# DrStiev/raytracing_rust

Hardware: AMD Instinct MI355X
Metric: Msamples/s (W×H×spp/s) + wall-clock to PPM, final_scene 1920×1080×1000spp (higher is better)
Workload: dtype f32; 1 GPU; final_scene 1920x1080x1000spp; per_gpu=1920x1080x1000spp-equivalent (tiles t % 1 == rank), scene_seed=1, render_seed=42, max_depth=50, flags=1

## Files before the change

### raytracing_rust_amd/csrc/rtmi_bvh_coop.hpp

```cpp
#pragma once
#include "rtmi_bvh.hpp"
#include "rtmi_rng.hpp"

#define COOP_NONE 0xffffffffu
#define RTMI_COOP_DUMMY_WORDS 128u
#define COOP_SENTINEL 0xffffffffffffffffull
__device__ __forceinline__ uint32_t f2sort(float f) {
    const uint32_t u = __float_as_uint(f);
    return (u & 0x80000000u) ? ~u : (u | 0x80000000u);
}
__device__ __forceinline__ float sort2f(uint32_t s) {
    return __uint_as_float((s & 0x80000000u) ? (s & 0x7fffffffu) : ~s);
}

struct CoopLds {
    uint32_t cap;
    bool ext, insd;
    constexpr uint32_t ctx() const { return 2u * cap; }
    constexpr uint32_t best() const { return ctx() + 64u * 12u; }
    constexpr uint32_t dummy() const { return best() + 128u; }
    constexpr uint32_t ring() const { return dummy() + RTMI_COOP_DUMMY_WORDS; }
    constexpr uint32_t park() const { return ring() + (ext ? 0u : RTMI_RNG_RING_WORDS); }
    constexpr uint32_t words() const { return park() + (insd ? RTMI_COOP_PARK_WORDS : 0u); }
};

struct CoopWork {
    uint32_t *wlds;
    int cap;
    uint2 *spill;
    int spill_cap;
};

#define RTMI_COOP_INLINE __forceinline__
template <bool PROF, bool EXT, bool W4, bool INST, bool QU = false>
__device__ __forceinline__ void coop_bvh_query(const DevScene &sc, int root, bool gated, float scale, bool active, const RayF &R,
                                               float time, float q_min, float q_max, const CoopWork &cw,
                                               bool &have, float &t_out, int &pf_out, bool &overflow,
                                               unsigned long long *prof, int slot) {
    const int lane = threadIdx.x & 63;
    uint32_t *wlds = cw.wlds;
    const int cap = cw.cap;
    uint2 *pool = reinterpret_cast<uint2 *>(wlds);
    const CoopLds lds{(uint32_t)cap, false, false};
    float4 *ctx = reinterpret_cast<float4 *>(wlds + lds.ctx());
    unsigned long long *best = reinterpret_cast<unsigned long long *>(wlds + lds.best());

    const unsigned long long m_act = __ballot(active);
    have = false;
    if (m_act == 0ull) return;
    best[lane] = COOP_SENTINEL;
    uint32_t cur = COOP_NONE;
    int ray = 0, cray = -1, aray = -1;
    float tent = 0.0f;
    RayF W;
    W.o = f3(0, 0, 0); W.d = f3(0, 0, 1); W.inv_d = f3(0, 0, 0); W.a = 1.0f; W.inv_a = 1.0f;
    float wtime = 0.0f, wqmin = 0.0f, wqmax = 0.0f, wmabs = 0.0f;
    if (active) {
        ctx[lane * 3 + 0] = make_float4(R.o.x, R.o.y, R.o.z, time);
        ctx[lane * 3 + 1] = make_float4(R.d.x, R.d.y, R.d.z, QU ? R.inv_a : q_min);
        ctx[lane * 3 + 2] = make_float4(R.inv_d.x, R.inv_d.y, R.inv_d.z, q_max);
        cur = (uint32_t)root; ray = lane; cray = lane;
        tent = q_min;
        W.o = R.o; W.d = R.d; W.inv_d = R.inv_d;
        wtime = time; wqmin = q_min; wqmax = q_max;
        if (QU) { W.a = R.a; W.inv_a = R.inv_a; aray = lane; }
        wmabs = scale * (1.0f / 8192.0f) *
                fminf(fminf(__builtin_fabsf(W.inv_d.x), __builtin_fabsf(W.inv_d.y)), __builtin_fabsf(W.inv_d.z));
    }
    if (QU) wqmin = q_min;
    int top = 0, gtop = 0;
    __builtin_amdgcn_fence(__ATOMIC_RELEASE, "wavefront");
    __builtin_amdgcn_wave_barrier();

    uint32_t wch[4] = {0u, 0u, 0u, 0u};
    float wtn[4] = {0.0f, 0.0f, 0.0f, 0.0f};
    const auto visit4 = [&](float limit, uint32_t &wkeep, int &npush) {
        const uint32_t base = cur * 8u;
        const uint32_t sx = W.inv_d.x < 0.0f ? 3u : 0u, sy = W.inv_d.y < 0.0f ? 3u : 0u, sz = W.inv_d.z < 0.0f ? 3u : 0u;
        const float4 nx4 = sc.nodes4[base + sx], fx4 = sc.nodes4[base + 3u - sx];
        const float4 ny4 = sc.nodes4[base + 1u + sy], fy4 = sc.nodes4[base + 4u - sy];
        const float4 nz4 = sc.nodes4[base + 2u + sz], fz4 = sc.nodes4[base + 5u - sz];
        const float4 chf = sc.nodes4[base + 6u];
        const float anx[4] = {nx4.x, nx4.y, nx4.z, nx4.w}, afx[4] = {fx4.x, fx4.y, fx4.z, fx4.w};
        const float any_[4] = {ny4.x, ny4.y, ny4.z, ny4.w}, afy[4] = {fy4.x, fy4.y, fy4.z, fy4.w};
        const float anz[4] = {nz4.x, nz4.y, nz4.z, nz4.w}, afz[4] = {fz4.x, fz4.y, fz4.z, fz4.w};
        wch[0] = __float_as_uint(chf.x); wch[1] = __float_as_uint(chf.y); wch[2] = __float_as_uint(chf.z); wch[3] = __float_as_uint(chf.w);
        int nearest = -1;
        float tnear = RTMI_FLT_MAX;
        const float far0 = fminf(wqmax, limit);
#pragma unroll
        for (int c = 0; c < 4; c++) {
            const float tn = fmaxf(fmaxf(fmaxf(wqmin, (anx[c] - W.o.x) * W.inv_d.x), (any_[c] - W.o.y) * W.inv_d.y), (anz[c] - W.o.z) * W.inv_d.z);
            const float tf = fminf(fminf(fminf(far0, (afx[c] - W.o.x) * W.inv_d.x), (afy[c] - W.o.y) * W.inv_d.y), (afz[c] - W.o.z) * W.inv_d.z);
            wtn[c] = tn;
            const bool okc = !(tn > tf) && wch[c] != COOP_NONE;
            if (okc) wkeep |= 1u << c;
            if (okc && !(tn >= tnear)) { nearest = c; tnear = tn; }
        }
        if (nearest >= 0) { cur = wch[nearest]; tent = tnear; wkeep &= ~(1u << nearest); } else cur = COOP_NONE;
        npush = __popc(wkeep);
    };
    const auto publish4 = [&](uint32_t wkeep, int npush) {
        const unsigned long long b0 = __ballot((npush & 1) != 0), b1 = __ballot((npush & 2) != 0);
        const int before = (int)__builtin_amdgcn_mbcnt_hi((uint32_t)(b0 >> 32), __builtin_amdgcn_mbcnt_lo((uint32_t)b0, 0u)) +
                           2 * (int)__builtin_amdgcn_mbcnt_hi((uint32_t)(b1 >> 32), __builtin_amdgcn_mbcnt_lo((uint32_t)b1, 0u));
        int at = top + before;
        const int dummy = cap + (int)((lds.dummy() - lds.ctx()) / 2u) + lane;
#pragma unroll
        for (int c = 0; c < 4; c++) {
            const bool on = (wkeep & (1u << c)) != 0u;
            pool[on ? at : dummy] = make_uint2(((uint32_t)ray << 26) | wch[c], __float_as_uint(wtn[c]));
            at += on ? 1 : 0;
        }
        top += __popcll(b0) + 2 * __popcll(b1);
    };
    for (;;) {
    for (;;) {
        const bool needw = cur == COOP_NONE;
        const unsigned long long m_need = __ballot(needw);
        const int n_need = __popcll(m_need);
        if (top == 0 && n_need == 64) break;
        if (top > cap - (W4 ? 192 : 64)) {
            if (!EXT) overflow = true;
            break;
        }
        const int take = n_need < top ? n_need : top;
        {
            const int r = (int)__builtin_amdgcn_mbcnt_hi((uint32_t)(m_need >> 32), __builtin_amdgcn_mbcnt_lo((uint32_t)m_need, 0u));
            if (needw && r < take) {
                const int idx = top - 1 - r;
                const uint2 e = pool[idx];
                tent = __uint_as_float(e.y);
                cur = e.x & 0x03ffffffu;
                ray = (int)(e.x >> 26);
            }
        }
        top -= take;
        prof_tick<PROF>(prof, slot, cur != COOP_NONE);
        bool push = false;
        uint32_t push_ref = 0u;
        float push_t = 0.0f;
        int npush = 0;
        uint32_t wkeep = 0u;
        {
            if (cur != COOP_NONE && ray != cray) {
                const float4 c0 = ctx[ray * 3 + 0], c1 = ctx[ray * 3 + 1], c2 = ctx[ray * 3 + 2];
                W.o = f3(c0.x, c0.y, c0.z); wtime = c0.w;
                W.d = f3(c1.x, c1.y, c1.z);
                if (QU) W.inv_a = c1.w; else wqmin = c1.w;
                W.inv_d = f3(c2.x, c2.y, c2.z); wqmax = c2.w;
                wmabs = scale * (1.0f / 8192.0f) *
                        fminf(fminf(__builtin_fabsf(W.inv_d.x), __builtin_fabsf(W.inv_d.y)), __builtin_fabsf(W.inv_d.z));
                cray = ray;
            }
            const unsigned long long key = best[ray];
            const float bt = sort2f((uint32_t)(key >> 32));
            const float lim = bt + (__builtin_fabsf(bt) * (1.0f / 128.0f) + wmabs);
            const float limit = key != COOP_SENTINEL ? lim : RTMI_FLT_MAX;
            if (tent > limit) cur = COOP_NONE;
            if (W4 && !(cur & (1u << 25))) {
                visit4(limit, wkeep, npush);
            } else if (!W4 && !(cur & (1u << 25))) {
                const float4 *n = sc.nodes + (size_t)cur * 4;
                const float4 n0 = n[0], n1 = n[1], n2 = n[2], n3 = n[3];
                const uint32_t left = __float_as_uint(n3.z), right = __float_as_uint(n3.w);
                float tl, tr;
                bool vl = aabb_hit_t(n0.x, n0.y, n0.z, n0.w, n1.x, n1.y, W, wqmin, wqmax, tl);
                bool vr = aabb_hit_t(n1.z, n1.w, n2.x, n2.y, n2.z, n2.w, W, wqmin, wqmax, tr);
                vl = vl && !(tl > limit);
                vr = vr && !(tr > limit) && right != left;
                if (vl && vr) {
                    const bool lfirst = !(tr < tl);
                    push = true;
                    push_ref = lfirst ? right : left;
                    push_t = lfirst ? tr : tl;
                    cur = lfirst ? left : right;
                    tent = lfirst ? tl : tr;
                } else if (vl) { cur = left; tent = tl; }
                else if (vr) { cur = right; tent = tr; }
                else cur = COOP_NONE;
            }
        }
        if (cur != COOP_NONE && (cur & (1u << 25))) {
            {
                const int type = (int)((cur >> 22) & 7u);
                const int idx = (int)(cur & 0x003fffffu);
                float t;
                int pf;
                if (type <= RTMI_PRIM_MSPHERE && aray != ray) {
                    W.a = dot(W.d, W.d);
                    if (!QU) W.inv_a = 1.0f / W.a;
                    aray = ray;
                }
                bool hit;
                if (EXT && gated) {
                    const float4 *rec = sc.leaf_rec + (size_t)idx * 5;
                    const float4 A = rec[0], B = rec[1], M = rec[2], g0 = rec[3], g1 = rec[4];
                    hit = prim_test_vals<INST>(sc, type, idx, A, B, M.z, __float_as_uint(M.y), W, wtime, wqmin, wqmax, t, pf);
                    if (hit) hit = aabb_hit(g0.x, g0.y, g0.z, g1.x, g1.y, g1.z, W, wqmin, wqmax);
                } else {
                    hit = prim_test<INST>(sc, type, idx, W, wtime, wqmin, wqmax, t, pf);
                }
                if (hit) {
                    const unsigned long long k = ((unsigned long long)f2sort(t) << 32) | (unsigned long long)(0x7fffffffu - (uint32_t)pf);
                    atomicMin(&best[ray], k);
                }
                cur = COOP_NONE;
            }
        }
        if (W4) {
            if (__ballot(npush != 0) != 0ull) publish4(wkeep, npush);
        } else {
        const unsigned long long m_push = __ballot(push);
        if (push) {
            const int pos = top + (int)__builtin_amdgcn_mbcnt_hi((uint32_t)(m_push >> 32), __builtin_amdgcn_mbcnt_lo((uint32_t)m_push, 0u));
            pool[pos] = make_uint2(((uint32_t)ray << 26) | push_ref, __float_as_uint(push_t));
        }
        top += __popcll(m_push);
        }
        if (PROF && lane == 0) atomicMax(&prof[2 * 18], (unsigned long long)top);
        __builtin_amdgcn_fence(__ATOMIC_ACQ_REL, "wavefront");
        __builtin_amdgcn_wave_barrier();
    }
        if (!EXT) break;
        if (top > cap - (W4 ? 192 : 64)) {
            const int m = top - 64;
            if (gtop + m > cw.spill_cap) { overflow = true; break; }
            for (int i = lane; i < m; i += 64) cw.spill[gtop + i] = pool[i];
            const int rest = top - m;
            for (int base = 0; base < rest; base += 64) {
                const int i = base + lane;
                uint2 e = make_uint2(0u, 0u);
                if (i < rest) e = pool[m + i];
                __builtin_amdgcn_wave_barrier();
                if (i < rest) pool[i] = e;
            }
            gtop += m;
            top = rest;
        } else if (gtop > 0) {
            const int n = gtop < cap / 2 ? gtop : cap / 2;
            for (int i = lane; i < n; i += 64) pool[i] = cw.spill[gtop - n + i];
            gtop -= n;
            top = n;
        } else {
            break;
        }
        __builtin_amdgcn_fence(__ATOMIC_ACQ_REL, "wavefront");
        __builtin_amdgcn_wave_barrier();
    }
    __builtin_amdgcn_fence(__ATOMIC_ACQ_REL, "wavefront");
    __builtin_amdgcn_wave_barrier();
    if (active) {
        const unsigned long long key = best[lane];
        if (key != COOP_SENTINEL) {
            have = true;
            t_out = sort2f((uint32_t)(key >> 32));
            pf_out = (int)(0x7fffffffu - (uint32_t)key);
        }
    }
    __builtin_amdgcn_wave_barrier();
}

template <bool PROF, bool EXT, bool W4, bool INST, bool ONE = false, bool QU = false>
__device__ __forceinline__ bool geom_query_coop(const DevScene &sc, const rtmi_item &I, bool use_alt, bool active, const RayF &r,
                                                float time, float q_min, float q_max, const CoopWork &cw,
                                                float &t_out, int &pf_out, bool &overflow, unsigned long long *prof,
                                                int slot) {
    if (I.kind == RTMI_ITEM_BVH) {
        const bool enter = active && aabb_hit(I.root_min[0], I.root_min[1], I.root_min[2], I.root_max[0], I.root_max[1],
                                              I.root_max[2], r, q_min, q_max);
        bool have = false;
        static_assert(!ONE || (EXT && W4), "the one-tree form walks the gated 4-wide tree");
        if constexpr (ONE) {
            coop_bvh_query<PROF, EXT, W4, INST, QU>(sc, I.alt_first, true, I.scale, enter, r, time, q_min, q_max, cw, have, t_out, pf_out, overflow, prof, slot);
        } else {
        const bool alt = EXT && W4 && use_alt && I.alt_first >= 0;
        if (alt) coop_bvh_query<PROF, EXT, W4, INST, QU>(sc, I.alt_first, true, I.scale, enter, r, time, q_min, q_max, cw, have, t_out, pf_out, overflow, prof, slot);
        else coop_bvh_query<PROF, EXT, false, INST, QU>(sc, I.first, false, I.scale, enter, r, time, q_min, q_max, cw, have, t_out, pf_out, overflow, prof, slot);
        }
        return have;
    }
    float cl = q_max;
    bool any = false;
    if (active) {
        for (int k = 0; k < I.count; k++) {
            const int idx = I.first + k;
            float t;
            int pf;
            prof_tick<PROF>(prof, 13, true);
            if (prim_test_uniform<INST>(sc, idx, r, time, q_min, cl, t, pf)) { cl = t; any = true; pf_out = pf; }
        }
    }
    t_out = cl;
    return any;
}
```

### raytracing_rust_amd/csrc/rtmi_device.hip

```cpp
#include <hip/hip_runtime.h>

#include <dlfcn.h>
#include <time.h>

#include <algorithm>
#include <cmath>
#include <cstdio>
#include <cstdlib>
#include <cstring>
#include <limits>
#include <map>
#include <mutex>
#include <new>
#include <string>
#include <thread>
#include <utility>
#include <vector>

#include "rtmi.h"
#include "rtmi_math.h"

#include "rtmi_kernels.hpp"
#include "rtmi_render_launch.hpp"
#include "rtmi_probe_path_launch.hpp"
// ... 178 lines not shown
    if (d->max_bvh_depth > RTMI_MAX_BVH_DEPTH)
        return fail(RTMI_ERR_UNSUPPORTED, "BVH deeper than RTMI_MAX_BVH_DEPTH");
    if (d->n_prims >= (1u << 28)) return fail(RTMI_ERR_UNSUPPORTED, "too many primitives");
    if ((d->n_prims && (!d->prim_a || !d->prim_b || !d->prim_meta)) || (d->n_nodes && !d->nodes) || (d->n_xforms && !d->xforms) ||
        (d->n_materials && !d->materials) || (d->n_textures && !d->textures) || (d->n_perlin && !d->perlin) ||
        (d->n_images && !d->images) || (d->image_bytes && !d->image_data))
        return fail(RTMI_ERR_INVALID, "a non-zero count comes with a NULL array");
    auto prim_ok = [&](int64_t i) { return i >= 0 && (uint64_t)i < d->n_prims; };
    for (uint32_t i = 0; i < d->n_prims; i++) {
        const rtmi_prim_meta &m = d->prim_meta[i];
        if (m.type < 0 || m.type > RTMI_PRIM_CUBE) return fail(RTMI_ERR_INVALID, "bad primitive type");
        if (m.material < 0 || (uint32_t)m.material >= d->n_materials)
            return fail(RTMI_ERR_INVALID, "primitive material out of range");
        const uint32_t xfc = (m.flags >> RTMI_PRIMFLAG_XF_COUNT_SHIFT) & RTMI_PRIM_XF_MAX, xff = m.flags >> RTMI_PRIMFLAG_XF_FIRST_SHIFT;
        if (xfc != 0u && ((uint64_t)xff + xfc > d->n_xforms)) return fail(RTMI_ERR_INVALID, "primitive transform range out of bounds");
        for (uint32_t k = 0; k < xfc; k++)
            if (d->xforms[xff + k].kind > RTMI_XF_ROTATE_Z) return fail(RTMI_ERR_INVALID, "a gate or inner-medium record inside a primitive's transform chain");
    }
    for (uint32_t i = 0; i < d->n_xforms; i++)
        if (d->xforms[i].kind < RTMI_XF_TRANSLATE || d->xforms[i].kind > RTMI_XF_INNER_MEDIUM) return fail(RTMI_ERR_INVALID, "bad transform kind");
    for (uint32_t i = 0; i < d->n_nodes; i++) {
        const int32_t ch[2] = {d->nodes[i].left, d->nodes[i].right};
        for (int c = 0; c < 2; c++) {
            if (ch[c] >= 0) {
                if ((uint32_t)ch[c] >= d->n_nodes) return fail(RTMI_ERR_INVALID, "BVH child out of range");
            } else {
                uint32_t type = ((uint32_t)ch[c] >> 28) & 7u, idx = (uint32_t)ch[c] & 0x0fffffffu;
                if (type > RTMI_PRIM_CUBE || !prim_ok(idx)) return fail(RTMI_ERR_INVALID, "BVH leaf out of range");
                if ((int)type != d->prim_meta[idx].type) return fail(RTMI_ERR_INVALID, "BVH leaf type mismatch");
            }
        }
    }
    if (d->n_alt_nodes && !d->alt_nodes) return fail(RTMI_ERR_INVALID, "n_alt_nodes without alt_nodes");
    for (uint32_t i = 0; i < d->n_alt_nodes; i++)
        for (int c = 0; c < 4; c++) {
            const int32_t ch = d->alt_nodes[i].child[c];
            if (ch == RTMI_NO_CHILD) continue;
            if (ch >= 0) {
                if ((uint32_t)ch >= d->n_alt_nodes) return fail(RTMI_ERR_INVALID, "alternative tree child out of range");
            } else {
                const uint32_t type = ((uint32_t)ch >> 28) & 7u, idx = (uint32_t)ch & 0x0fffffffu;
                if (type > RTMI_PRIM_CUBE || !prim_ok(idx)) return fail(RTMI_ERR_INVALID, "alternative tree leaf out of range");
                if ((int)type != d->prim_meta[idx].type) return fail(RTMI_ERR_INVALID, "alternative tree leaf type mismatch");
            }
        }
    std::vector<uint8_t> seen_bin(d->n_nodes, 0), seen_alt(d->n_alt_nodes, 0);
    std::vector<std::pair<uint32_t, uint32_t>> todo;
    const auto walk = [&](bool alt, uint32_t root, uint32_t declared, const char *what) -> int {
        std::vector<uint8_t> &seen = alt ? seen_alt : seen_bin;
        todo.clear();
        todo.emplace_back(root, 1u);
        while (!todo.empty()) {
            const uint32_t n = todo.back().first, depth = todo.back().second;
            todo.pop_back();
            if (seen[n]) return fail(RTMI_ERR_INVALID, std::string(what) + ": a node is reached twice (cycle or shared subtree)");
            seen[n] = 1;
            if (depth > declared) return fail(RTMI_ERR_INVALID, std::string(what) + " is deeper than the declared depth");
            if (alt) {
                for (int c = 0; c < 4; c++) {
                    const int32_t ch = d->alt_nodes[n].child[c];
                    if (ch >= 0 && ch != RTMI_NO_CHILD) todo.emplace_back((uint32_t)ch, depth + 1u);
                }
            } else {
                const int32_t l = d->nodes[n].left, r = d->nodes[n].right;
                if (l >= 0) todo.emplace_back((uint32_t)l, depth + 1u);
                if (r >= 0 && r != l) todo.emplace_back((uint32_t)r, depth + 1u);
// ... 514 lines not shown
    hipStream_t stream = reinterpret_cast<hipStream_t>(stream_);
    if (s->busy_recorded) HIP_TRY(hipStreamWaitEvent(stream, s->busy.e, 0));
    BusyMark busy_mark{s, stream};

    DevParams P = dev_params(s, p);
    if (P.ntiles_local == 0) {
        if (stats) memset(stats, 0, sizeof(*stats));
        return RTMI_OK;
    }
    P.path_sig = reinterpret_cast<unsigned long long *>(p->path_sig);
    if (p->flags & RTMI_FLAG_PATH_SIG) {
        if (!p->path_sig) return fail(RTMI_ERR_INVALID, "RTMI_FLAG_PATH_SIG needs params.path_sig");
        HIP_TRY(hipMemsetAsync(P.path_sig, 0, (size_t)P.ntiles_local * 64 * sizeof(unsigned long long), stream));
    }

    uint32_t chunk_spp = 0, pass_ns = 0;
    rc = plan_and_reserve(s, p, P.ntiles_local, chunk_spp, pass_ns);
    if (rc) return rc;
    P.chunk_spp = chunk_spp;
    P.pass_stride = pass_ns;
    P.samples = s->samples.ptr;
    const DevCamera C = dev_camera(cam);

    if (stats) HIP_TRY(hipEventRecord(s->ev[0].e, stream));
    const bool fast = (p->flags & RTMI_FLAG_FAST_CULL) != 0u && boxes_valid(s, cam), sigf = (p->flags & RTMI_FLAG_PATH_SIG) != 0u;
    const size_t dyn_lds = (size_t)WAVES_PER_BLOCK * 2u * P.stack_depth * 64u * sizeof(uint32_t);
    const bool prof = (p->flags & RTMI_FLAG_PROFILE) != 0u, sync = (p->flags & RTMI_FLAG_SYNC) != 0u;
    if (prof) {
        if (!p->prof) return fail(RTMI_ERR_INVALID, "RTMI_FLAG_PROFILE needs params.prof");
        P.prof = reinterpret_cast<unsigned long long *>(p->prof);
        HIP_TRY(hipMemsetAsync(P.prof, 0, 2 * RTMI_PROF_SLOTS * sizeof(unsigned long long), stream));
    }
    const bool async = (p->flags & RTMI_FLAG_ASYNC) != 0u && !s->has_deferred;
    const bool coop_ok = s->meta.n_prims < (1u << 22) && s->meta.n_nodes < (1u << 25) && s->meta.n_alt_nodes < (1u << 25);
    const bool coop = fast && !sync && !async && coop_ok;
    if ((rc = begin_passes(s, stream))) return rc;
    bool ext = false;
    if ((rc = plan_traversal(s, p, coop, P, ext))) return rc;
    if (p->flags & (1u << 11)) {
        ext = true;
        P.coop_cap = 256u;
    }
    const uint32_t wps_req = (p->flags >> 8) & 7u;
    const bool inst = s->dev.has_prim_xf != 0u || s->dev.has_medium_outer != 0u;
    const uint32_t wps_run = (coop && !prof && !sigf && !inst && (wps_req == 3u || wps_req == 5u)) ? wps_req : (coop && prof ? 3u : 4u);
    const uint64_t run_slots = (uint64_t)(s->slots / 20) * 4u * wps_run;
    const bool bcoop = coop && (p->flags & RTMI_FLAG_BLOCK_COOP) != 0u && P.use_alt && s->all_alt && !prof && !inst &&
                       wps_req == 0u;
    const size_t bcoop_lds = (size_t)RTMI_BLK_LDS_WORDS(RTMI_BLK_CAP) * sizeof(uint32_t);
    if (bcoop) P.coop_cap = (p->flags & (1u << 11)) ? 3u * RTMI_BLK_THREADS + 64u : RTMI_BLK_CAP;
    s->last_kernel = bcoop ? RTMI_KERNEL_BLOCK_COOP : coop ? RTMI_KERNEL_WAVE_COOP : async ? RTMI_KERNEL_ASYNC : RTMI_KERNEL_PERLANE;
    const bool one_tree = coop && !bcoop && ext && !inst && !sigf && !prof && wps_req == 0u && P.use_alt != 0u &&
                          !(p->flags & RTMI_FLAG_REF_TREE) && s->all_alt && s->all_sphere_media;
    s->last_inst = !coop || bcoop ? RTMI_INST_NONE : one_tree ? RTMI_INST_COOP_ONE_TREE : RTMI_INST_COOP_GENERAL;
    const bool insd = inst && (s->needs_insd || ext || sigf);
    const size_t coop_lds = (size_t)WAVES_PER_BLOCK * CoopLds{P.coop_cap, ext, insd}.words() * sizeof(uint32_t);
    const uint64_t max_blocks = async ? ~0ull : bcoop ? run_slots / RTMI_BLK_WAVES : run_slots;
    const RenderLaunch launch{bcoop, coop, async, inst, insd, prof, sigf, fast, ext, one_tree, wps_req, coop_lds, bcoop_lds, dyn_lds};
    PassCounts counts;
    rc = run_passes(s, P, stream, 0, p->ns, true, max_blocks, async ? WAVES_PER_BLOCK : 1u, counts,
                    [&](uint32_t blocks, bool first, bool last) -> int {
                        if (!bcoop && coop && inst && prof) return fail(RTMI_ERR_UNSUPPORTED, "the profiling build has no instantiation for instanced primitives / media inside transforms");
                        HIP_TRY(rtmi_render_launch(launch, blocks, stream, s->dev, C, P));
                        if (stats && last) HIP_TRY(hipEventRecord(s->ev[1].e, stream));
                        HIP_TRY(rtmi_render_launch_resolve(stream, s->samples.ptr, s->partial.ptr, reinterpret_cast<rtmi_texel *>(d_texels), P,
                                                           first, last, (p->flags & RTMI_FLAG_PROGRESSIVE) != 0u));
                        return RTMI_OK;
// ... 733 lines not shown
    if (m.env && !s->has_env)
        return fail(RTMI_ERR_INVALID, std::string(m.name) + ": no environment map attached (rtmi_scene_attach_env)");
    if (m.nee && !s->has_lights) return fail(RTMI_ERR_INVALID, std::string(m.name) + ": " + m.no_lights);
    return RTMI_OK;
}
int check_attached_early(const Estimator &m, const rtmi_scene *s_in) {
    if (!s_in) return RTMI_OK;
    rtmi_scene *s = const_cast<rtmi_scene *>(s_in);
    std::lock_guard<std::mutex> lock(s->mu);
    return check_attached(m, s);
}
int begin_call(RenderCall &c, const Estimator &m, rtmi_scene *s) {
    if (!s) return fail(RTMI_ERR_INVALID, m.null_scene);
    c.lock = std::unique_lock<std::mutex>(s->mu);
    if (int rc = check_attached(m, s)) return rc;
    if (m.tree && !s->has_light_tree)
        return fail(RTMI_ERR_INVALID, std::string(m.name) + ": no light tree attached (rtmi_scene_attach_light_tree)");
    HIP_TRY(hipSetDevice(s->device));
    if (int rc = begin_blocking(s)) return rc;
    c.busy.s = s; c.busy.st = s->stream.s;
    return RTMI_OK;
}
void kernel_args(RenderCall &c, const Estimator &m, const rtmi_scene *s, const rtmi_camera *cam,
                        const rtmi_render_params &p) {
    c.P = dev_params(s, &p);
    c.C = dev_camera(cam);
    c.fast = (p.flags & RTMI_FLAG_FAST_CULL) != 0u && boxes_valid(s, cam);
    dev_lighting(s, m.nee, m.env, m.env_select_p, c.L, c.E);
}
static uint32_t light_coop_bits(const rtmi_render_params *p, uint32_t flag = RTMI_FLAG_LIGHT_COOP) {
    return (p && (p->flags & flag)) ? (flag | (1u << 11)) : 0u;
}
int plan_light_coop(RenderCall &c, rtmi_scene *s, const rtmi_render_params &p, uint32_t flag, uint32_t wps) {
    const bool coop_ok = s->meta.n_prims < (1u << 22) && s->meta.n_nodes < (1u << 25) && s->meta.n_alt_nodes < (1u << 25);
    const bool inst = s->dev.has_prim_xf != 0u || s->dev.has_medium_outer != 0u;
    c.coop = (p.flags & flag) != 0u && c.fast && !(p.flags & RTMI_FLAG_SYNC) && coop_ok && !inst;
    if (!c.coop) return RTMI_OK;
    c.wps = wps;
    if (int rc = plan_traversal(s, &p, true, c.P, c.ext)) return rc;
    if (p.flags & (1u << 11)) {
        c.ext = true;
        c.P.coop_cap = 256u;
    }
    c.coop_lds = (size_t)WAVES_PER_BLOCK * CoopLds{c.P.coop_cap, c.ext, false}.words() * sizeof(uint32_t);
    return RTMI_OK;
}
uint64_t light_run_slots(const rtmi_scene *s, const RenderCall &c) {
    return (uint64_t)(s->slots / 20) * 4u * c.wps;
}
int launch_light_coop(const RenderCall &c, const Estimator &m, rtmi_scene *s, bool sig, uint32_t blocks, const uint32_t *tiles) {
    HIP_TRY(rtmi_light_coop_launch_render(tiles != nullptr, sig, c.ext, m.nee, m.env, blocks, c.coop_lds, s->stream.s, s->dev, c.C,
                                          c.P, tiles, c.L, c.E));
    return RTMI_OK;
}
static int begin_adaptive(RenderCall &c, const Estimator &m, rtmi_scene *s, const rtmi_camera *cam, const rtmi_render_params &p,
                          const rtmi_adaptive *a) {
    int rc;
    if ((rc = begin_call(c, m, s)) || (rc = adaptive_reserve(s, p, a, local_tiles_of(&p, 0)))) return rc;
    kernel_args(c, m, s, cam, p);
    return RTMI_OK;
}

template <typename Launch>
static int render_fixed_device(RenderCall &c, const Estimator &m, rtmi_scene *s, const rtmi_camera *cam, const rtmi_render_params &p,
                               bool sig, rtmi_stats *stats, Launch &&launch) {
    int rc;
    hipStream_t stream = s->stream.s;
// ... 28 lines not shown
        A.first = first ? 1 : 0;
        A.decide = last ? 1 : 0;
        if (last) HIP_TRY(hipMemsetAsync(A.n_out, 0, sizeof(uint32_t), stream));
        HIP_TRY(rtmi_adaptive_launch_resolve(stream, s->samples.ptr, P, A));
        return RTMI_OK;
    });
    if (rc) return rc;
    HIP_TRY(hipEventRecord(s->ev[2].e, stream));
    rtmi_scene *one[1] = {s};
    if ((rc = wait_with_progress(one, &s->ev[2].e, 1, &p))) return rc;
    if ((rc = check_overflow(s))) return rc;
    return stats ? fill_stats_from_events(s, &p, stats, counts) : RTMI_OK;
}
template <typename Launch>
static int render_fixed(const Estimator &m, rtmi_scene *s, const rtmi_camera *cam, const rtmi_render_params &p, float *out_linear,
                        uint8_t *out_rgb8, float *out_stderr, uint64_t *out_path_sig, rtmi_stats *stats, Launch &&launch) {
    RenderCall c;
    int rc;
    if ((rc = begin_call(c, m, s)) || (rc = render_fixed_device(c, m, s, cam, p, out_path_sig != nullptr, stats, launch))) return rc;
    const size_t ntex = (size_t)local_tiles_of(&p, 0) * 64;
    HIP_TRY(hipMemcpy(s->h_texels.ptr, s->texels.ptr, ntex * sizeof(rtmi_texel), hipMemcpyDeviceToHost));
    if (out_stderr && (rc = download_untiled<3>(&p, s->ad_stderr.ptr, ntex, out_stderr))) return rc;
    if (out_path_sig && (rc = download_untiled<1>(&p, s->d_sig.ptr, ntex, out_path_sig))) return rc;
    return rtmi_untile(&p, s->h_texels.ptr, out_linear, out_rgb8);
}

static int adaptive_plain_device(RenderCall &c, const Estimator &m, rtmi_scene *s, const rtmi_camera *cam, const rtmi_render_params &p,
                                 const rtmi_adaptive *a, PassCounts &counts) {
    int rc;
    if ((rc = adaptive_reserve(s, p, a, local_tiles_of(&p, 0)))) return rc;
    kernel_args(c, m, s, cam, p);
    DevParams &P = c.P;
    const bool fast = c.fast, sync = (p.flags & RTMI_FLAG_SYNC) != 0u;
    const bool coop_ok = s->meta.n_prims < (1u << 22) && s->meta.n_nodes < (1u << 25) && s->meta.n_alt_nodes < (1u << 25);
    const bool inst = s->dev.has_prim_xf != 0u || s->dev.has_medium_outer != 0u;
    const bool coop = fast && !sync && coop_ok && !inst;
    bool ext = false;
    if ((rc = plan_traversal(s, &p, coop, P, ext))) return rc;
    const int which = coop ? (ext ? RTMI_AD_COOP_EXT : RTMI_AD_COOP_LEAN) : (fast ? RTMI_AD_PERLANE_FAST : RTMI_AD_PERLANE);
    const size_t coop_lds = (size_t)WAVES_PER_BLOCK * CoopLds{P.coop_cap, ext, false}.words() * sizeof(uint32_t);
    return adaptive_steps_device(s, p, a, P, coop ? RTMI_KERNEL_WAVE_COOP : RTMI_KERNEL_PERLANE, 4u, counts,
                                 [&](uint32_t blocks, const uint32_t *tiles) -> int {
                                     HIP_TRY(rtmi_adaptive_launch_render(which, blocks, coop ? coop_lds : 0, s->stream.s, s->dev, c.C,
                                                                         P, tiles));
                                     return RTMI_OK;
                                 });
}

extern "C" int rtmi_render_adaptive(rtmi_scene *s, const rtmi_camera *cam, const rtmi_render_params *p_in,
                                    const rtmi_adaptive *a, float *out_linear, uint8_t *out_rgb8, float *out_stderr,
                                    uint32_t *out_spp, rtmi_stats *stats) {
    if (!p_in || !a || !cam) return fail(RTMI_ERR_INVALID, "NULL argument");
    int rc = check_mode_params(p_in, RTMI_FLAG_FAST_CULL | RTMI_FLAG_SYNC | RTMI_FLAG_REF_TREE | RTMI_FLAG_SKY | RTMI_FLAG_FACE_FORWARD |
                                         RTMI_FLAG_UV_BOOK,
                               "adaptive sampling accepts the flags FAST_CULL, SYNC, REF_TREE, SKY, FACE_FORWARD and "
                               "UV_BOOK only (not PATH_SIG, PROFILE, ASYNC, BLOCK_COOP, PROGRESSIVE, TEST_OVERFLOW)",
                               "adaptive sampling renders the whole image: tile_world must be 1");
    if (rc) return rc;
    if ((rc = check_adaptive(p_in, a))) return rc;
    const Estimator m{"rtmi_render_adaptive", false, false, 1.0f, "scene is NULL", ""};
    RenderCall c;
    PassCounts counts;
    if ((rc = begin_call(c, m, s)) || (rc = adaptive_plain_device(c, m, s, cam, *p_in, a, counts))) return rc;
    return adaptive_download(s, *p_in, counts, out_linear, out_rgb8, out_stderr, out_spp, stats);
}

static int features_device(rtmi_scene *s, const rtmi_camera *cam, const rtmi_render_params &p, bool sig, rtmi_stats *stats) {
// ... 670 lines not shown
```

### raytracing_rust_amd/csrc/rtmi_kernel_coop.inc

```
#ifndef RTMI_COOP_TAKE
#define RTMI_COOP_TAKE "rtmi_path_take.inc"
#define RTMI_COOP_TAKE_DEFAULTED
#endif
#ifndef RTMI_COOP_T_MIN
#define RTMI_COOP_T_MIN t_min
#define RTMI_COOP_T_MAX RTMI_FLT_MAX
#define RTMI_COOP_T_DEFAULTED
#endif
#ifdef RTMI_COOP_T_DEFAULTED
    constexpr bool T_MIN_UNIFORM = true;
#else
    constexpr bool T_MIN_UNIFORM = false;
#endif
    constexpr bool INST = INSTL >= 1;
    constexpr bool INSD = INSTL >= 2;
    constexpr bool FEATURES = false;
    __shared__ unsigned long long prof_lds[PROF ? 2 * RTMI_PROF_SLOTS : 1];
    unsigned long long *prof = prof_lds;
    if (PROF) {
        if (threadIdx.x < 2 * RTMI_PROF_SLOTS) prof_lds[threadIdx.x] = 0ull;
        __syncthreads();
    }
    extern __shared__ __attribute__((aligned(16))) uint32_t lds_dyn[];
    const int lane = threadIdx.x & 63;
// ... 106 lines not shown
                            if (reach && h1 && h2 && medium_sample<T_MIN_UNIFORM>(t1, t2, RTMI_COOP_T_MIN, t0_saved, medium_dir_norm<INST>(sc, I.flags, I.xform_first, W), I.neg_inv_density, g, k0, k1, tm)) {
                                if (scan) { park[64] = __float_as_uint(tm); park[128] = it | 0x80000000u; }
                                else if (tm < closest) { closest = tm; best_item = (int)it; best_medium = true; }
                            }
                            h1 = false;
                        }
                    }
                    if (need && h1 && h2) {
                        if (medium_sample<T_MIN_UNIFORM>(t1, t2, RTMI_COOP_T_MIN, closest, medium_dir_norm<INST>(sc, I.flags, I.xform_first, W), I.neg_inv_density, g, k0, k1, tm)) {
                            closest = tm; best_item = (int)it; best_medium = true;
                        }
                    }
                    prof_time<PROF>(prof, 29, tstamp);
                }
            }
            if (need) {
#include "rtmi_path_traced.inc"
            }
            if (__popcll(__ballot(have_hit)) >= threshold) break;
        }
#define RTMI_PATH_SCRATCH cw.wlds
#define RTMI_PATH_INST INST
#include "rtmi_path_shade.inc"
#undef RTMI_PATH_SCRATCH
#undef RTMI_PATH_INST
        prof_time<PROF>(prof, 30, tstamp);
    }
    if (P.ext & RTMI_EXT_TEST_OVERFLOW) overflow = true;
    if (__ballot(overflow) != 0ull && lane == 0) atomicAdd(P.status, 1u);

    if (PROF) {
        __syncthreads();
        if (threadIdx.x < 2 * RTMI_PROF_SLOTS && prof_lds[threadIdx.x] != 0ull) {
            if (threadIdx.x == 2 * 18) atomicMax(P.prof + threadIdx.x, prof_lds[threadIdx.x]);
            else atomicAdd(P.prof + threadIdx.x, prof_lds[threadIdx.x]);
        }
    }
#ifdef RTMI_COOP_TAKE_DEFAULTED
#undef RTMI_COOP_TAKE
#undef RTMI_COOP_TAKE_DEFAULTED
#endif
#ifdef RTMI_COOP_T_DEFAULTED
#undef RTMI_COOP_T_MIN
#undef RTMI_COOP_T_MAX
#undef RTMI_COOP_T_DEFAULTED
#endif
```

### raytracing_rust_amd/csrc/rtmi_prof.hpp

```cpp
#pragma once
#include "rtmi_types.hpp"

#define RTMI_PROF_SLOTS 32
template <bool PROF>
__device__ __forceinline__ void prof_tick(unsigned long long *prof_lds, int slot, bool active) {
    if (PROF) {
        const unsigned long long m = __ballot(active);
        if (m != 0ull && (int)(__ffsll((long long)m) - 1) == (int)(threadIdx.x & 63)) {
            atomicAdd(&prof_lds[2 * slot], (unsigned long long)__popcll(m));
            atomicAdd(&prof_lds[2 * slot + 1], 64ull);
        }
    }
}

template <bool PROF>
__device__ __forceinline__ void prof_time(unsigned long long *prof_lds, int slot, unsigned long long &t_prev) {
    if (PROF) {
        const unsigned long long t = __builtin_readcyclecounter();
        if ((threadIdx.x & 63) == 0) {
            atomicAdd(&prof_lds[2 * slot], t - t_prev);
            atomicAdd(&prof_lds[2 * slot + 1], 1ull);
        }
        t_prev = __builtin_readcyclecounter();
    }
}
```

### raytracing_rust_amd/csrc/rtmi_types.hpp

```cpp
#pragma once
#include <cstddef>
#include <hip/hip_runtime.h>

#include <cstdint>

#include "rtmi.h"
#include "rtmi_math.h"

#define RTMI_FLT_MAX 3.40282346638528859811704183484516925e+38f
#define WAVES_PER_BLOCK 1

struct F3 {
    float x, y, z;
};
__device__ __forceinline__ F3 f3(float x, float y, float z) { return F3{x, y, z}; }
__device__ __forceinline__ F3 operator+(F3 a, F3 b) { return f3(a.x + b.x, a.y + b.y, a.z + b.z); }
__device__ __forceinline__ F3 operator-(F3 a, F3 b) { return f3(a.x - b.x, a.y - b.y, a.z - b.z); }
__device__ __forceinline__ F3 operator-(F3 a) { return f3(-a.x, -a.y, -a.z); }
__device__ __forceinline__ F3 operator*(F3 a, float s) { return f3(a.x * s, a.y * s, a.z * s); }
__device__ __forceinline__ F3 operator*(F3 a, F3 b) { return f3(a.x * b.x, a.y * b.y, a.z * b.z); }
__device__ __forceinline__ F3 vdiv(F3 a, float s) { return f3(a.x / s, a.y / s, a.z / s); }
__device__ __forceinline__ float dot(F3 a, F3 b) { return a.x * b.x + a.y * b.y + a.z * b.z; }
__device__ __forceinline__ float norm(F3 a) { return __builtin_sqrtf(dot(a, a)); }
__device__ __forceinline__ F3 normalize(F3 a) { return vdiv(a, norm(a)); }
template <int I>
__device__ __forceinline__ float comp(F3 a) {
    return I == 0 ? a.x : (I == 1 ? a.y : a.z);
}

struct DevItem {
    rtmi_item it;
    rtmi_xform x0, x1;
};
static_assert(sizeof(rtmi_item) == 64 && sizeof(rtmi_xform) == 16 && sizeof(DevItem) == 96, "DevItem layout");
static_assert(offsetof(rtmi_item, flags) == 12 && offsetof(rtmi_item, medium_material) == 24, "item shading words at bytes 12..27");
static_assert(offsetof(DevItem, x0) == 64 && offsetof(DevItem, x1) == 80, "embedded transforms at bytes 64 and 80");

struct PrimRec {
    float4 A, B;
    rtmi_prim_meta M;
};
static_assert(sizeof(PrimRec) == 48, "leaf record head");

struct DevScene {
    const DevItem *items;
    const float4 *prim_a;
    const float4 *prim_b;
    const rtmi_prim_meta *meta;
    const float4 *gate;
    const float4 *nodes;
    const float4 *nodes4;
    const float4 *shade_prim;
    const float4 *shade_mat;
    const float4 *leaf_rec;
    const rtmi_xform *xforms;
    const rtmi_material *mats;
    const rtmi_texture *texs;
    const rtmi_perlin *perlin;
    const rtmi_image *images;
    const uint8_t *image_data;
    uint32_t n_items;
    uint32_t has_prim_xf;
    uint32_t has_medium_outer;
};

struct Rad3 { float r, g, b; };
static_assert(sizeof(Rad3) == RTMI_SAMPLE_SLOT_BYTES, "per-sample slot size is part of rtmi.h");

struct DevCamera {
// ... 33 lines not shown
```

Measured before the change: 2665 Msamples/s.

## Add quad-lane cooperative BVH rounds and byte-offset node loads

```diff
diff --git a/raytracing_rust_amd/csrc/rtmi_bvh_coop.hpp b/raytracing_rust_amd/csrc/rtmi_bvh_coop.hpp
--- a/raytracing_rust_amd/csrc/rtmi_bvh_coop.hpp
+++ b/raytracing_rust_amd/csrc/rtmi_bvh_coop.hpp
@@ -5,6 +5,10 @@
 #define COOP_NONE 0xffffffffu
 #define RTMI_COOP_DUMMY_WORDS 128u
 #define COOP_SENTINEL 0xffffffffffffffffull
+#ifndef RTMI_COOP_QUAD_MAX
+#define RTMI_COOP_QUAD_MAX 16
+#endif
+static_assert(RTMI_COOP_QUAD_MAX >= 0 && RTMI_COOP_QUAD_MAX <= 16, "a quad round gives every entry four of the 64 lanes");
 __device__ __forceinline__ uint32_t f2sort(float f) {
     const uint32_t u = __float_as_uint(f);
     return (u & 0x80000000u) ? ~u : (u | 0x80000000u);
@@ -32,7 +36,7 @@
 };
 
 #define RTMI_COOP_INLINE __forceinline__
-template <bool PROF, bool EXT, bool W4, bool INST, bool QU = false>
+template <bool PROF, bool EXT, bool W4, bool INST, bool QU = false, bool SP = false>
 __device__ __forceinline__ void coop_bvh_query(const DevScene &sc, int root, bool gated, float scale, bool active, const RayF &R,
                                                float time, float q_min, float q_max, const CoopWork &cw,
                                                bool &have, float &t_out, int &pf_out, bool &overflow,
@@ -75,12 +79,23 @@
     uint32_t wch[4] = {0u, 0u, 0u, 0u};
     float wtn[4] = {0.0f, 0.0f, 0.0f, 0.0f};
     const auto visit4 = [&](float limit, uint32_t &wkeep, int &npush) {
-        const uint32_t base = cur * 8u;
-        const uint32_t sx = W.inv_d.x < 0.0f ? 3u : 0u, sy = W.inv_d.y < 0.0f ? 3u : 0u, sz = W.inv_d.z < 0.0f ? 3u : 0u;
-        const float4 nx4 = sc.nodes4[base + sx], fx4 = sc.nodes4[base + 3u - sx];
-        const float4 ny4 = sc.nodes4[base + 1u + sy], fy4 = sc.nodes4[base + 4u - sy];
-        const float4 nz4 = sc.nodes4[base + 2u + sz], fz4 = sc.nodes4[base + 5u - sz];
-        const float4 chf = sc.nodes4[base + 6u];
+        float4 nx4, fx4, ny4, fy4, nz4, fz4, chf;
+        if constexpr (SP) {
+            const uint32_t boff = cur << 7;
+            const uint32_t ox = boff + (W.inv_d.x < 0.0f ? 48u : 0u), oy = boff + (W.inv_d.y < 0.0f ? 48u : 0u),
+                           oz = boff + (W.inv_d.z < 0.0f ? 48u : 0u);
+            nx4 = gather16(sc.nodes4, ox); fx4 = gather16(sc.nodes4, ox ^ 48u);
+            ny4 = gather16<16u>(sc.nodes4, oy); fy4 = gather16<16u>(sc.nodes4, oy ^ 48u);
+            nz4 = gather16<32u>(sc.nodes4, oz); fz4 = gather16<32u>(sc.nodes4, oz ^ 48u);
+            chf = gather16<96u>(sc.nodes4, boff);
+        } else {
+            const uint32_t base = cur * 8u;
+            const uint32_t sx = W.inv_d.x < 0.0f ? 3u : 0u, sy = W.inv_d.y < 0.0f ? 3u : 0u, sz = W.inv_d.z < 0.0f ? 3u : 0u;
+            nx4 = sc.nodes4[base + sx]; fx4 = sc.nodes4[base + 3u - sx];
+            ny4 = sc.nodes4[base + 1u + sy]; fy4 = sc.nodes4[base + 4u - sy];
+            nz4 = sc.nodes4[base + 2u + sz]; fz4 = sc.nodes4[base + 5u - sz];
+            chf = sc.nodes4[base + 6u];
+        }
         const float anx[4] = {nx4.x, nx4.y, nx4.z, nx4.w}, afx[4] = {fx4.x, fx4.y, fx4.z, fx4.w};
         const float any_[4] = {ny4.x, ny4.y, ny4.z, ny4.w}, afy[4] = {fy4.x, fy4.y, fy4.z, fy4.w};
         const float anz[4] = {nz4.x, nz4.y, nz4.z, nz4.w}, afz[4] = {fz4.x, fz4.y, fz4.z, fz4.w};
@@ -114,7 +129,33 @@
         }
         top += __popcll(b0) + 2 * __popcll(b1);
     };
+    const auto visit1 = [&](float limit, uint32_t &wkeep) {
+        const uint32_t boff = (cur << 7) + 4u * ((uint32_t)lane & 3u);
+        const uint32_t ox = boff + (W.inv_d.x < 0.0f ? 48u : 0u), oy = boff + (W.inv_d.y < 0.0f ? 48u : 0u),
+                       oz = boff + (W.inv_d.z < 0.0f ? 48u : 0u);
+        const float nx = gather4(sc.nodes4, ox), fx = gather4(sc.nodes4, ox ^ 48u);
+        const float ny = gather4<16u>(sc.nodes4, oy), fy = gather4<16u>(sc.nodes4, oy ^ 48u);
+        const float nz = gather4<32u>(sc.nodes4, oz), fz = gather4<32u>(sc.nodes4, oz ^ 48u);
+        const uint32_t ch = __float_as_uint(gather4<96u>(sc.nodes4, boff));
+        const float far0 = fminf(wqmax, limit);
+        const float tn = fmaxf(fmaxf(fmaxf(wqmin, (nx - W.o.x) * W.inv_d.x), (ny - W.o.y) * W.inv_d.y), (nz - W.o.z) * W.inv_d.z);
+        const float tf = fminf(fminf(fminf(far0, (fx - W.o.x) * W.inv_d.x), (fy - W.o.y) * W.inv_d.y), (fz - W.o.z) * W.inv_d.z);
+        const bool okc = !(tn > tf) && ch != COOP_NONE;
+        const bool leaf = (ch & (1u << 25)) != 0u;
+        wch[0] = ch; wtn[0] = tn;
+        wkeep = (okc && !leaf) ? 1u : 0u;
+        cur = (okc && leaf) ? ch : COOP_NONE;
+    };
+    const auto publish1 = [&](uint32_t wkeep) {
+        const unsigned long long b0 = __ballot(wkeep != 0u);
+        const int at = (int)__builtin_amdgcn_mbcnt_hi((uint32_t)(b0 >> 32), __builtin_amdgcn_mbcnt_lo((uint32_t)b0, 0u));
+        const int dummy = cap + (int)((lds.dummy() - lds.ctx()) / 2u) + lane;
+        pool[wkeep != 0u ? at : dummy] = make_uint2(((uint32_t)ray << 26) | wch[0], __float_as_uint(wtn[0]));
+        top = __popcll(b0);
+    };
+    constexpr bool QUADS = SP && W4 && EXT && RTMI_COOP_QUAD_MAX > 0;
     for (;;) {
+    const int qmax = gtop == 0 ? RTMI_COOP_QUAD_MAX : -1;
     for (;;) {
         const bool needw = cur == COOP_NONE;
         const unsigned long long m_need = __ballot(needw);
@@ -124,8 +165,33 @@
             if (!EXT) overflow = true;
             break;
         }
-        const int take = n_need < top ? n_need : top;
-        {
+        bool quad = false;
+        if constexpr (QUADS) quad = 64 - n_need + top <= qmax;
+        int busy;
+        if (quad) {
+            if (!needw) {
+                const unsigned long long m_hold = ~m_need;
+                const int r = (int)__builtin_amdgcn_mbcnt_hi((uint32_t)(m_hold >> 32), __builtin_amdgcn_mbcnt_lo((uint32_t)m_hold, 0u));
+                pool[top + r] = make_uint2(((uint32_t)ray << 26) | cur, __float_as_uint(tent));
+            }
+            busy = top + 64 - n_need;
+            __builtin_amdgcn_fence(__ATOMIC_ACQ_REL, "wavefront");
+            __builtin_amdgcn_wave_barrier();
+            cur = COOP_NONE;
+            if ((lane >> 2) < busy) {
+                const uint2 e = pool[busy - 1 - (lane >> 2)];
+                tent = __uint_as_float(e.y);
+                cur = e.x & 0x03ffffffu;
+                ray = (int)(e.x >> 26);
+                if ((cur & (1u << 25)) && (lane & 3) != 0) cur = COOP_NONE;
+            }
+            top = 0;
+            if (PROF && RTMI_PROF_ROUND_COUNTERS && lane == 0) {
+                atomicAdd(&prof[RTMI_PROF_QUAD_ROUNDS], 1ull);
+                atomicMax(&prof[RTMI_PROF_QUAD_MAX_ENTRIES], (unsigned long long)busy);
+            }
+        } else {
+            const int take = n_need < top ? n_need : top;
             const int r = (int)__builtin_amdgcn_mbcnt_hi((uint32_t)(m_need >> 32), __builtin_amdgcn_mbcnt_lo((uint32_t)m_need, 0u));
             if (needw && r < take) {
                 const int idx = top - 1 - r;
@@ -134,9 +200,14 @@
                 cur = e.x & 0x03ffffffu;
                 ray = (int)(e.x >> 26);
             }
-        }
-        top -= take;
+            top -= take;
+            busy = 64 - n_need + take;
+        }
         prof_tick<PROF>(prof, slot, cur != COOP_NONE);
+        if (PROF && RTMI_PROF_ROUND_COUNTERS && lane == 0) {
+            const int bucket = busy <= 4 ? 0 : busy <= 8 ? 1 : busy <= 16 ? 2 : busy <= 32 ? 3 : 4;
+            atomicAdd(&prof[RTMI_PROF_ROUND_HIST + (slot == 1 ? 0 : RTMI_PROF_ROUND_BUCKETS) + bucket], 1ull);
+        }
         bool push = false;
         uint32_t push_ref = 0u;
         float push_t = 0.0f;
@@ -159,7 +230,8 @@
             const float limit = key != COOP_SENTINEL ? lim : RTMI_FLT_MAX;
             if (tent > limit) cur = COOP_NONE;
             if (W4 && !(cur & (1u << 25))) {
-                visit4(limit, wkeep, npush);
+                if (quad) visit1(limit, wkeep);
+                else visit4(limit, wkeep, npush);
             } else if (!W4 && !(cur & (1u << 25))) {
                 const float4 *n = sc.nodes + (size_t)cur * 4;
                 const float4 n0 = n[0], n1 = n[1], n2 = n[2], n3 = n[3];
@@ -194,8 +266,15 @@
                 }
                 bool hit;
                 if (EXT && gated) {
-                    const float4 *rec = sc.leaf_rec + (size_t)idx * 5;
-                    const float4 A = rec[0], B = rec[1], M = rec[2], g0 = rec[3], g1 = rec[4];
+                    float4 A, B, M, g0, g1;
+                    if constexpr (SP) {
+                        const uint32_t loff = (uint32_t)idx * 80u;
+                        A = gather16(sc.leaf_rec, loff); B = gather16<16u>(sc.leaf_rec, loff); M = gather16<32u>(sc.leaf_rec, loff);
+                        g0 = gather16<48u>(sc.leaf_rec, loff); g1 = gather16<64u>(sc.leaf_rec, loff);
+                    } else {
+                        const float4 *rec = sc.leaf_rec + (size_t)idx * 5;
+                        A = rec[0]; B = rec[1]; M = rec[2]; g0 = rec[3]; g1 = rec[4];
+                    }
                     hit = prim_test_vals<INST>(sc, type, idx, A, B, M.z, __float_as_uint(M.y), W, wtime, wqmin, wqmax, t, pf);
                     if (hit) hit = aabb_hit(g0.x, g0.y, g0.z, g1.x, g1.y, g1.z, W, wqmin, wqmax);
                 } else {
@@ -209,7 +288,8 @@
             }
         }
         if (W4) {
-            if (__ballot(npush != 0) != 0ull) publish4(wkeep, npush);
+            if (quad) publish1(wkeep);
+            else if (__ballot(npush != 0) != 0ull) publish4(wkeep, npush);
         } else {
         const unsigned long long m_push = __ballot(push);
         if (push) {
@@ -272,10 +352,10 @@
         bool have = false;
         static_assert(!ONE || (EXT && W4), "the one-tree form walks the gated 4-wide tree");
         if constexpr (ONE) {
-            coop_bvh_query<PROF, EXT, W4, INST, QU>(sc, I.alt_first, true, I.scale, enter, r, time, q_min, q_max, cw, have, t_out, pf_out, overflow, prof, slot);
+            coop_bvh_query<PROF, EXT, W4, INST, QU, true>(sc, I.alt_first, true, I.scale, enter, r, time, q_min, q_max, cw, have, t_out, pf_out, overflow, prof, slot);
         } else {
         const bool alt = EXT && W4 && use_alt && I.alt_first >= 0;
-        if (alt) coop_bvh_query<PROF, EXT, W4, INST, QU>(sc, I.alt_first, true, I.scale, enter, r, time, q_min, q_max, cw, have, t_out, pf_out, overflow, prof, slot);
+        if (alt) coop_bvh_query<PROF, EXT, W4, INST, QU, PROF>(sc, I.alt_first, true, I.scale, enter, r, time, q_min, q_max, cw, have, t_out, pf_out, overflow, prof, slot);
         else coop_bvh_query<PROF, EXT, false, INST, QU>(sc, I.first, false, I.scale, enter, r, time, q_min, q_max, cw, have, t_out, pf_out, overflow, prof, slot);
         }
         return have;
diff --git a/raytracing_rust_amd/csrc/rtmi_device.hip b/raytracing_rust_amd/csrc/rtmi_device.hip
--- a/raytracing_rust_amd/csrc/rtmi_device.hip
+++ b/raytracing_rust_amd/csrc/rtmi_device.hip
@@ -234,6 +234,7 @@
         }
     }
     if (d->n_alt_nodes && !d->alt_nodes) return fail(RTMI_ERR_INVALID, "n_alt_nodes without alt_nodes");
+    if (d->n_alt_nodes >= (1u << 25)) return fail(RTMI_ERR_UNSUPPORTED, "too many alternative tree nodes");
     for (uint32_t i = 0; i < d->n_alt_nodes; i++)
         for (int c = 0; c < 4; c++) {
             const int32_t ch = d->alt_nodes[i].child[c];
@@ -814,7 +815,7 @@
         HIP_TRY(hipMemsetAsync(P.prof, 0, 2 * RTMI_PROF_SLOTS * sizeof(unsigned long long), stream));
     }
     const bool async = (p->flags & RTMI_FLAG_ASYNC) != 0u && !s->has_deferred;
-    const bool coop_ok = s->meta.n_prims < (1u << 22) && s->meta.n_nodes < (1u << 25) && s->meta.n_alt_nodes < (1u << 25);
+    const bool coop_ok = s->meta.n_prims < (1u << 22) && s->meta.n_nodes < (1u << 25);
     const bool coop = fast && !sync && !async && coop_ok;
     if ((rc = begin_passes(s, stream))) return rc;
     bool ext = false;
@@ -1614,7 +1615,7 @@
     return (p && (p->flags & flag)) ? (flag | (1u << 11)) : 0u;
 }
 int plan_light_coop(RenderCall &c, rtmi_scene *s, const rtmi_render_params &p, uint32_t flag, uint32_t wps) {
-    const bool coop_ok = s->meta.n_prims < (1u << 22) && s->meta.n_nodes < (1u << 25) && s->meta.n_alt_nodes < (1u << 25);
+    const bool coop_ok = s->meta.n_prims < (1u << 22) && s->meta.n_nodes < (1u << 25);
     const bool inst = s->dev.has_prim_xf != 0u || s->dev.has_medium_outer != 0u;
     c.coop = (p.flags & flag) != 0u && c.fast && !(p.flags & RTMI_FLAG_SYNC) && coop_ok && !inst;
     if (!c.coop) return RTMI_OK;
@@ -1709,7 +1710,7 @@
     kernel_args(c, m, s, cam, p);
     DevParams &P = c.P;
     const bool fast = c.fast, sync = (p.flags & RTMI_FLAG_SYNC) != 0u;
-    const bool coop_ok = s->meta.n_prims < (1u << 22) && s->meta.n_nodes < (1u << 25) && s->meta.n_alt_nodes < (1u << 25);
+    const bool coop_ok = s->meta.n_prims < (1u << 22) && s->meta.n_nodes < (1u << 25);
     const bool inst = s->dev.has_prim_xf != 0u || s->dev.has_medium_outer != 0u;
     const bool coop = fast && !sync && coop_ok && !inst;
     bool ext = false;
diff --git a/raytracing_rust_amd/csrc/rtmi_kernel_coop.inc b/raytracing_rust_amd/csrc/rtmi_kernel_coop.inc
--- a/raytracing_rust_amd/csrc/rtmi_kernel_coop.inc
+++ b/raytracing_rust_amd/csrc/rtmi_kernel_coop.inc
@@ -162,7 +162,7 @@
     if (PROF) {
         __syncthreads();
         if (threadIdx.x < 2 * RTMI_PROF_SLOTS && prof_lds[threadIdx.x] != 0ull) {
-            if (threadIdx.x == 2 * 18) atomicMax(P.prof + threadIdx.x, prof_lds[threadIdx.x]);
+            if (threadIdx.x == 2 * 18 || threadIdx.x == RTMI_PROF_QUAD_MAX_ENTRIES) atomicMax(P.prof + threadIdx.x, prof_lds[threadIdx.x]);
             else atomicAdd(P.prof + threadIdx.x, prof_lds[threadIdx.x]);
         }
     }
diff --git a/raytracing_rust_amd/csrc/rtmi_prof.hpp b/raytracing_rust_amd/csrc/rtmi_prof.hpp
--- a/raytracing_rust_amd/csrc/rtmi_prof.hpp
+++ b/raytracing_rust_amd/csrc/rtmi_prof.hpp
@@ -2,6 +2,13 @@
 #include "rtmi_types.hpp"
 
 #define RTMI_PROF_SLOTS 32
+#define RTMI_PROF_ROUND_HIST (2 * 20)
+#define RTMI_PROF_ROUND_BUCKETS 5
+#define RTMI_PROF_QUAD_ROUNDS (2 * 17)
+#define RTMI_PROF_QUAD_MAX_ENTRIES (2 * 19)
+#ifndef RTMI_PROF_ROUND_COUNTERS
+#define RTMI_PROF_ROUND_COUNTERS 1
+#endif
 template <bool PROF>
 __device__ __forceinline__ void prof_tick(unsigned long long *prof_lds, int slot, bool active) {
     if (PROF) {
diff --git a/raytracing_rust_amd/csrc/rtmi_types.hpp b/raytracing_rust_amd/csrc/rtmi_types.hpp
--- a/raytracing_rust_amd/csrc/rtmi_types.hpp
+++ b/raytracing_rust_amd/csrc/rtmi_types.hpp
@@ -35,6 +35,16 @@
 static_assert(sizeof(rtmi_item) == 64 && sizeof(rtmi_xform) == 16 && sizeof(DevItem) == 96, "DevItem layout");
 static_assert(offsetof(rtmi_item, flags) == 12 && offsetof(rtmi_item, medium_material) == 24, "item shading words at bytes 12..27");
 static_assert(offsetof(DevItem, x0) == 64 && offsetof(DevItem, x1) == 80, "embedded transforms at bytes 64 and 80");
+
+template <uint32_t IMM = 0u>
+__device__ __forceinline__ float4 gather16(const float4 *base, uint32_t off) {
+    return *reinterpret_cast<const float4 *>(reinterpret_cast<const char *>(base) + (uint64_t)off + IMM);
+}
+
+template <uint32_t IMM = 0u>
+__device__ __forceinline__ float gather4(const float4 *base, uint32_t off) {
+    return *reinterpret_cast<const float *>(reinterpret_cast<const char *>(base) + (uint64_t)off + IMM);
+}
 
 struct PrimRec {
     float4 A, B;
```

After: 2723 Msamples/s, median of 6. 2.2% higher.
